# google-research/weatherbenchX

Measured on AMD Instinct MI355X. Metric: grid-point·metric evals/s (0.25° 721×1440×37L) at 1/2/4/8 GPUs; % HBM roofline, higher is better.
Workload: dtype f32+f64

## Files before the change

### weatherbenchx_amd/csrc/wbx_common.hpp

```cpp
#pragma once
#include <hip/hip_runtime.h>

#include <cstdarg>
#include <cstdint>
#include <cstdio>
#include <cstring>

#include "../../include/wbx.h"

struct wbx_ctx {
  int device = 0;
  int num_cus = 256;
  hipStream_t stream = nullptr;
  bool own_stream = false;
  hipEvent_t ev_start = nullptr;
  hipEvent_t ev_stop = nullptr;
  void* fft_state = nullptr;
  void* s2_scratch = nullptr;
  size_t s2_scratch_size = 0;
  void* aidm_scratch = nullptr;
  size_t aidm_scratch_size = 0;
  void* atoms_clean = nullptr;
  void* patch_counters = nullptr;
  size_t patch_counters_size = 0;
  uint32_t ens_queue_parity = 0;
  hipEvent_t* marks = nullptr;
  int marks_used = 0, marks_made = 0, marks_cap = 0;
};

namespace wbx {

char* last_error_buf();

inline int fail(int code, const char* fmt, ...) {
  va_list ap;
  va_start(ap, fmt);
  vsnprintf(last_error_buf(), 512, fmt, ap);
  va_end(ap);
  return code;
}

template <typename T>
__device__ __forceinline__ T ld_stream(const T* p) {
#ifdef WBX_LD_STREAM_PLAIN
  return *p;
#else
  return __builtin_nontemporal_load(p);
#endif
}

__device__ __forceinline__ const char* uniform_ptr(const char* p) {
  const uint64_t v = (uint64_t)p;
  const uint32_t lo = __builtin_amdgcn_readfirstlane((uint32_t)v), hi = __builtin_amdgcn_readfirstlane((uint32_t)(v >> 32));
  return (const char*)(((uint64_t)hi << 32) | lo);
}

template <typename T>
using global_ptr = const __attribute__((address_space(1))) T*;

template <typename T>
using const_ptr = const __attribute__((address_space(4))) T*;

static __constant__ int64_t wbx_zero_i64[1] = {0};
static __constant__ double wbx_one_f64[1] = {1.0};

__device__ __forceinline__ int64_t readlane64(int64_t v, int j) {
  const int lo = __builtin_amdgcn_readlane((int)(uint32_t)(uint64_t)v, j);
  const int hi = __builtin_amdgcn_readlane((int)(uint32_t)((uint64_t)v >> 32), j);
  return (int64_t)(((uint64_t)(uint32_t)hi << 32) | (uint32_t)lo);
}

__device__ __forceinline__ double wave_sum(double v) {
#pragma unroll
  for (int o = 32; o > 0; o >>= 1) v += __shfl_xor(v, o, 64);
  return v;
}

template <int CTRL, int ROW_MASK>
__device__ __forceinline__ double dpp_moved(double v) {
  const int lo = __builtin_amdgcn_update_dpp(0, __double2loint(v), CTRL, ROW_MASK, 0xf, true);
  const int hi = __builtin_amdgcn_update_dpp(0, __double2hiint(v), CTRL, ROW_MASK, 0xf, true);
  return __hiloint2double(hi, lo);
}

__device__ __forceinline__ double wave_sum_lane63(double v) {
  v += dpp_moved<0xB1, 0xf>(v);
  v += dpp_moved<0x4E, 0xf>(v);
  v += dpp_moved<0x124, 0xf>(v);
  v += dpp_moved<0x128, 0xf>(v);
  v += dpp_moved<0x142, 0xa>(v);
  v += dpp_moved<0x143, 0xc>(v);
  return v;
}

__device__ __forceinline__ double wave_sum_uniform(double v) {
  const double t = wave_sum_lane63(v);
  return __hiloint2double(__builtin_amdgcn_readlane(__double2hiint(t), 63), __builtin_amdgcn_readlane(__double2loint(t), 63));
}

}

#define WBX_HIP(expr)                                                                   \
  do {                                                                                  \
    hipError_t _e = (expr);                                                             \
    if (_e != hipSuccess)                                                               \
      return wbx::fail(WBX_ERR_HIP, "%s failed: %s (%s:%d)", #expr, hipGetErrorString(_e), \
                       __FILE__, __LINE__);                                             \
  } while (0)

#define WBX_REQUIRE(cond, ...)                                   \
  do {                                                           \
    if (!(cond)) return wbx::fail(WBX_ERR_INVALID, __VA_ARGS__); \
  } while (0)
```

### weatherbenchx_amd/csrc/wbx_ens_impl.hpp

```cpp
#pragma once
#include <cmath>
#include <cstdlib>

#include "wbx_s1.hpp"
#include "wbx_sortnet_gen.hpp"
#include "wbx_sortnet3_gen.hpp"

#ifndef WBX_ENS_MIN_WAVES
#define WBX_ENS_MIN_WAVES 1
#endif

#ifndef WBX_ENS_MIN_WAVES_PLAIN
#define WBX_ENS_MIN_WAVES_PLAIN WBX_ENS_MIN_WAVES
#endif
#ifndef WBX_ENS_SORTNET3
#define WBX_ENS_SORTNET3 1
#endif

#ifndef WBX_ENS_NOFALLBACK
#define WBX_ENS_NOFALLBACK 0
#endif
#ifndef WBX_ENS_STATS32
#define WBX_ENS_STATS32 1
#endif

namespace wbx {

constexpr int WBX_ENS_DIAG_LOADONLY = 99;
constexpr int WBX_ENS_DIAG_PAIRWISE_LDS = 98;
constexpr int WBX_ENS_SKIPNA_SORT = 97;

template <typename T>
struct EnsOpGeneric {
  static constexpr int NIN = 2;
  static constexpr int NLANE = WBX_ENS_LANES;
  static constexpr int NACC = WBX_ENS_LANES;
  static constexpr int XR_UNROLL = 1, XK_UNROLL = 1, MIN_WAVES = 1;

  __device__ __forceinline__ static void values(const S1Args& a, const int64_t (&ro)[WBX_MAX_INPUTS], int64_t x,
                                                double (&val)[NLANE]) {
    const int M = a.M;
    const T* pp = reinterpret_cast<const T*>(a.in[0]) + ro[0] + x * a.xstride[0];
    const double td = (double)(reinterpret_cast<const T*>(a.in[1])[ro[1] + x * a.xstride[1]]);
    const bool skip = a.flags & WBX_FLAG_SKIPNA_ENS;
    double se = 0.0, sq = 0.0, sabs = 0.0, pair_total = 0.0, x0 = 0.0;
    int n = 0;
    for (int i = 0; i < M; ++i) {
      const double xi = (double)pp[(int64_t)i * a.mstride];
      if (skip && xi != xi) continue;
      if (n == 0) x0 = xi;
      ++n;
      const double e = xi - x0;
      se += e;
      sq = fma(e, e, sq);
      sabs += fabs(xi - td);
      double row = 0.0;
      for (int j = 0; j < i; ++j) {
        const double xj = (double)pp[(int64_t)j * a.mstride];
        if (skip && xj != xj) continue;
        row += fabs(xi - xj);
      }
      pair_total += row;
    }
    const double dM = (double)n;
    const double fair = (a.flags & WBX_FLAG_FAIR) ? 1.0 : 0.0;
    const double mean_e = se / dM;
    const double mean_d = (x0 - td) + mean_e;
    const double var = (sq - se * mean_e) / (dM - 1.0);
    val[0] = sabs / dM;
    val[1] = 2.0 * pair_total / (dM * (dM - fair));
    val[2] = var;
    val[3] = mean_d * mean_d - var / dM;
    val[4] = mean_d * mean_d;
  }

  template <int V, bool XK>
  __device__ __forceinline__ static void accum(const S1Args& a, const int64_t (&ro)[WBX_MAX_INPUTS], int64_t x,
                                               double (&acc)[XK ? V : 1][NACC]) {
    static_assert(V == 1, "ensemble op is one point per lane");
    double val[NLANE];
    values(a, ro, x, val);
#pragma unroll
    for (int l = 0; l < NLANE; ++l) acc[0][l] += val[l];
  }
};

template <int MP, bool EXACT, int ALGO>
struct EnsOpF32 {
  static constexpr int NIN = 2;
  static constexpr int NLANE = WBX_ENS_LANES;
  static constexpr int NACC = WBX_ENS_LANES;
  static constexpr int XR_UNROLL = 1, XK_UNROLL = 1, MIN_WAVES = WBX_ENS_MIN_WAVES_PLAIN;

  struct Regs {
    float xm[MP];
    float t;
    float poison;
  };

  __device__ __forceinline__ static void load(const S1Args& a, const int64_t (&ro)[WBX_MAX_INPUTS], int64_t x, Regs& r) {
    const int M = EXACT ? MP : a.M;
    const float* pp = reinterpret_cast<const float*>(a.in[0]) + ro[0] + x * a.xstride[0];
    r.t = ld_stream(reinterpret_cast<const float*>(a.in[1]) + ro[1] + x * a.xstride[1]);
#pragma unroll
    for (int m = 0; m < MP; ++m) r.xm[m] = (EXACT || m < M) ? ld_stream(pp + (int64_t)m * a.mstride) : INFINITY;
  }

  __device__ __forceinline__ static void values(const S1Args& a, const int64_t (&ro)[WBX_MAX_INPUTS], int64_t x,
                                                double (&val)[NLANE]) {
    Regs r;
    load(a, ro, x, r);
    finish(a, ro, x, r, val);
  }

  template <bool FAST32 = false>
  __device__ __forceinline__ static bool compute(const S1Args& a, Regs& r, double (&val)[NLANE]) {
    const int M = EXACT ? MP : a.M;
    const double td = (double)r.t;
    float(&xm)[MP] = r.xm;

    if constexpr (ALGO == WBX_ENS_DIAG_LOADONLY) {
      float s = 0.f;
#pragma unroll
      for (int m = 0; m < MP; ++m)
        if (EXACT || m < M) s += xm[m];
      val[0] = (double)s - td;
      val[1] = val[2] = val[3] = val[4] = 0.0;
      return false;
    }
    double pair_total = 0.0;
    float poison = 0.f;
    int nvalid = 0;
    bool weird = false;
    float shift32 = 0.f;
    if constexpr (ALGO == WBX_ENS_SKIPNA_SORT) {
      const bool tfin32 = (r.t - r.t) == 0.f;
      shift32 = r.t;
      if (__builtin_amdgcn_ballot_w64(!tfin32)) {
        float lo = INFINITY;
#pragma unroll
        for (int m = 0; m < MP; ++m)
          if (EXACT || m < M) lo = fminf(lo, xm[m]);
        shift32 = tfin32 ? r.t : lo;
      }
#pragma unroll
      for (int m = 0; m < MP; ++m) {
        if (EXACT || m < M) {
          const float x = xm[m];
          const bool missing = x != x;
          nvalid += missing ? 0 : 1;
          xm[m] = missing ? shift32 : x;
        }
      }
      if constexpr (!EXACT) {
        float big = 0.f;
        int m = 0;
        for (; m + 1 < MP; m += 2) {
          const float a = m < M ? xm[m] : 0.f, b = m + 1 < M ? xm[m + 1] : 0.f;
          asm("v_max3_f32 %0, %1, |%2|, |%3|" : "=v"(big) : "v"(big), "v"(a), "v"(b));
        }
        if (m < MP) {
          const float a = m < M ? xm[m] : 0.f;
          asm("v_max3_f32 %0, %1, |%2|, |%2|" : "=v"(big) : "v"(big), "v"(a));
        }
        weird = big == INFINITY;
      }
    }
    if constexpr (ALGO == WBX_ENS_PAIRWISE) {
#pragma unroll
      for (int i = 1; i < MP; ++i) {
        if (EXACT || i < M) {
          float row = 0.f;
#pragma unroll
          for (int j = 0; j < i; ++j) row += fabsf(xm[i] - xm[j]);
          pair_total += (double)row;
        }
      }
    } else if constexpr (ALGO == WBX_ENS_SORT || ALGO == WBX_ENS_SKIPNA_SORT) {
      if constexpr (ALGO == WBX_ENS_SORT) {
        typedef float pk2 __attribute__((ext_vector_type(2)));
        pk2 pz = {0.f, 0.f};
#pragma unroll
        for (int m = 0; m + 1 < MP; m += 2) {
          const pk2 x2 = {xm[m], (EXACT || m + 1 < M) ? xm[m + 1] : 0.f};
          if (EXACT || m < M) pz = x2 * (pk2){0.f, 0.f} + pz;
        }
        if ((MP & 1) && (EXACT || MP - 1 < M)) pz.x = fmaf(xm[MP - 1], 0.f, pz.x);
        poison = pz.x + pz.y;
      }
      auto mn = [](float u, float v) {
        float r;
        asm("v_min_f32 %0, %1, %2" : "=v"(r) : "v"(u), "v"(v));
        return r;
      };
      auto mx = [](float u, float v) {
        float r;
        asm("v_max_f32 %0, %1, %2" : "=v"(r) : "v"(u), "v"(v));
        return r;
      };
      if constexpr (WBX_ENS_SORTNET3) {
        SortNet3<MP>::sort(
            xm, mn, mx,
            [](float u, float v, float w) {
              float r;
              asm("v_min3_f32 %0, %1, %2, %3" : "=v"(r) : "v"(u), "v"(v), "v"(w));
              return r;
            },
            [](float u, float v, float w) {
              float r;
              asm("v_med3_f32 %0, %1, %2, %3" : "=v"(r) : "v"(u), "v"(v), "v"(w));
              return r;
            },
            [](float u, float v, float w) {
              float r;
              asm("v_max3_f32 %0, %1, %2, %3" : "=v"(r) : "v"(u), "v"(v), "v"(w));
              return r;
            });
      } else {
        SortNet<MP>::sort(xm, mn, mx);
      }
    }

    bool redo = false;
    if constexpr (ALGO == WBX_ENS_SKIPNA_SORT) {
      if constexpr (EXACT) weird = xm[0] == -INFINITY || xm[MP - 1] == INFINITY;
      stats_skipna(a, xm, nvalid, td, shift32, val);
      r.poison = 0.f;
      return weird;
    }
    if constexpr (FAST32 && EXACT && ALGO == WBX_ENS_SORT && WBX_ENS_STATS32) {
      const float range = xm[MP - 1] - xm[0];
      const float big = fmaxf(fmaxf(fabsf(xm[0]), fabsf(xm[MP - 1])), fabsf(r.t));
      const bool fast_ok = (range == 0.f || (range >= 0x1p-50f && range <= 0x1p60f)) && big <= 0x1p100f;
      redo = !WBX_ENS_NOFALLBACK && __builtin_amdgcn_ballot_w64(!fast_ok) != 0;
      if (!redo) stats32(a, xm, r.t, poison, val);
      r.poison = poison;
    } else {
      stats64(a, xm, td, pair_total, val);
      r.poison = poison;
      apply_poison(r, val);
    }
    return redo;
  }

  __device__ __forceinline__ static void apply_poison(const Regs& r, double (&val)[NLANE]) {
    if constexpr (ALGO == WBX_ENS_SORT) {
      if (r.poison != r.poison) {
#pragma unroll
        for (int l = 0; l < NLANE; ++l) val[l] = (double)r.poison;
      }
    }
  }

  template <bool FAST32 = false>
  __device__ __forceinline__ static void finish(const S1Args& a, const int64_t (&ro)[WBX_MAX_INPUTS], int64_t x, Regs& r,
                                                double (&val)[NLANE]) {
    if (compute<FAST32>(a, r, val)) {
      EnsOpGeneric<float>::values(a, ro, x, val);
      apply_poison(r, val);
    }
  }

  __device__ __forceinline__ static double recip_small(double n) {
    double r = __builtin_amdgcn_rcp(n);
    r = fma(fma(-n, r, 1.0), r, r);
    r = fma(fma(-n, r, 1.0), r, r);
    return r;
  }
  __device__ __forceinline__ static void stats_skipna(const S1Args& a, const float (&xm)[MP], const int n, const double td,
                                                      const float shift32, double (&val)[NLANE]) {
    const int M = EXACT ? MP : a.M;
    const double shift = (double)shift32;
    const double x0t = shift - td;
    const double dM = (double)n, dK = (double)(M - n);
    double se = 0.0, sq = 0.0, sabs = 0.0, dot1 = 0.0;
#pragma unroll
    for (int m = 0; m < MP; ++m) {
      if (EXACT || m < M) {
        const double e = (double)xm[m] - shift;
        se += e;
        sq = fma(e, e, sq);
        sabs += fabs(e);
        dot1 = fma((double)(2 * m + 1), e, dot1);
      }
    }
    const double dot = fma(-dM, se, fma(-dK, sabs + se, dot1));
    sabs += n > 0 ? fabs(x0t) : 0.0;
    const double nan = __builtin_nan("");
    const double inv_n = n > 0 ? recip_small(dM) : nan;
    const double inv_n1 = n > 1 ? recip_small(dM - 1.0) : nan;
    const double inv_pairs = (a.flags & WBX_FLAG_FAIR) ? inv_n * inv_n1 : inv_n * inv_n;
    const double mean_e = se * inv_n;
    const double mean_d = x0t + mean_e;
    const double var = (sq - se * mean_e) * inv_n1;
    val[0] = sabs * inv_n;
    val[1] = 2.0 * dot * inv_pairs;
    val[2] = var;
    val[3] = mean_d * mean_d - var * inv_n;
    val[4] = mean_d * mean_d;
  }

  __device__ __forceinline__ static void stats64(const S1Args& a, float (&xm)[MP], const double td, const double pair_total,
                                                 double (&val)[NLANE]) {
    const int M = EXACT ? MP : a.M;
    const double x0 = (double)xm[0];
    const bool tfin = (td - td) == 0.0;
    const double shift = tfin ? td : x0;
    const double x0t = shift - td;
    double se = 0.0, sq = 0.0, sabs = 0.0, dot = 0.0;
#pragma unroll
    for (int m = 0; m < MP; ++m) {
      if (EXACT || m < M) {
        const double e = (double)xm[m] - shift;
        se += e;
        sq = fma(e, e, sq);
        sabs += fabs(e);
        if constexpr (ALGO == WBX_ENS_SORT) dot = fma((double)(2 * (m + 1) - M - 1), e, dot);
      }
    }
    sabs += fabs(x0t);
    const double dM = (double)M;
    const double fair = (a.flags & WBX_FLAG_FAIR) ? 1.0 : 0.0;
    const double inv_m = 1.0 / dM, inv_m1 = 1.0 / (dM - 1.0), spread_scale = 2.0 / (dM * (dM - fair));
    const double mean_e = se * inv_m;
    const double mean_d = x0t + mean_e;
    const double var = (sq - se * mean_e) * inv_m1;
    double spread;
    if constexpr (ALGO == WBX_ENS_SORT) {
      spread = dot * spread_scale;
    } else {
      spread = pair_total * spread_scale;
    }
    if constexpr (ALGO == WBX_ENS_DIAG_PAIRWISE_LDS) {
      static_assert(EXACT && MP % 17 == 0, "the LDS-tiled diagnostic is instantiated for M = 51");
      constexpr int B = 17, NB = MP / B;
      __shared__ float tile[MP][64];
      float* col = &tile[0][threadIdx.x];
#pragma unroll
      for (int m = 0; m < MP; ++m) col[m * 64] = xm[m];
      asm volatile("" ::: "memory");
      double total = 0.0;
#pragma unroll
      for (int bi = 0; bi < NB; ++bi) {
        float xi[B];
#pragma unroll
        for (int k = 0; k < B; ++k) xi[k] = col[(bi * B + k) * 64];
#pragma unroll
        for (int k = 1; k < B; ++k) {
          float row = 0.f;
#pragma unroll
          for (int l = 0; l < k; ++l) row += fabsf(xi[k] - xi[l]);
          total += (double)row;
        }
#pragma unroll
        for (int bj = 0; bj < bi; ++bj) {
          float xj[B];
#pragma unroll
          for (int l = 0; l < B; ++l) xj[l] = col[(bj * B + l) * 64];
#pragma unroll
          for (int k = 0; k < B; ++k) {
            float row = 0.f;
#pragma unroll
            for (int l = 0; l < B; ++l) row += fabsf(xi[k] - xj[l]);
            total += (double)row;
          }
        }
      }
      spread = total * spread_scale;
    }
    val[0] = sabs * inv_m;
    val[1] = spread;
    val[2] = var;
    val[3] = mean_d * mean_d - var * inv_m;
    val[4] = mean_d * mean_d;
  }

  __device__ __forceinline__ static void stats32(const S1Args& a, float (&xm)[MP], const float t, const float poison,
                                                 double (&val)[NLANE]) {
    static_assert(EXACT, "fp32 chain sums are instantiated for the exact-M buckets");
    constexpr int K = 8, MID = MP / 2, NPAIR = MP / 2;
    const float c = xm[MID];
    float se[K], sq[K], sa[K], dt[K];
#pragma unroll
    for (int k = 0; k < K; ++k) se[k] = sq[k] = sa[k] = dt[k] = k == 0 ? poison : 0.f;
#pragma unroll
    for (int i = 0; i < NPAIR; ++i) {
      const int j = MP - 1 - i, k = i % K;
      const float ei = xm[i] - c, ej = xm[j] - c;
      se[k] += ei + ej;
      sq[k] = fmaf(ei, ei, sq[k]);
      sq[k] = fmaf(ej, ej, sq[k]);
      sa[k] += fabsf(xm[i] - t);
      sa[k] += fabsf(xm[j] - t);
      dt[k] = fmaf((float)(MP - 1 - 2 * i), xm[j] - xm[i], dt[k]);
    }
    if constexpr (MP & 1) {
      sa[NPAIR % K] += fabsf(c - t);
    } else {
    }
    auto fold = [](const float (&v)[K]) {
      return ((double)(v[0] + v[4]) + (double)(v[1] + v[5])) + ((double)(v[2] + v[6]) + (double)(v[3] + v[7]));
    };
    const double dse = fold(se), dsq = fold(sq), dsa = fold(sa), ddt = fold(dt);
    constexpr double dM = (double)MP;
    const double fair = (a.flags & WBX_FLAG_FAIR) ? 1.0 : 0.0;
    constexpr double inv_m = 1.0 / dM, inv_m1 = 1.0 / (dM - 1.0);
    const double spread_scale = 2.0 / (dM * (dM - fair));
    const double mean_e = dse * inv_m;
    const double mean_d = ((double)c - (double)t) + mean_e;
    const double var = (dsq - dse * mean_e) * inv_m1;
    val[0] = dsa * inv_m;
    val[1] = ddt * spread_scale;
    val[2] = var;
    val[3] = mean_d * mean_d - var * inv_m;
    val[4] = mean_d * mean_d;
  }

  template <int V, bool XK>
  __device__ __forceinline__ static void accum(const S1Args& a, const int64_t (&ro)[WBX_MAX_INPUTS], int64_t x,
                                               double (&acc)[XK ? V : 1][NACC]) {
    static_assert(V == 1, "ensemble op is one point per lane");
    double val[NLANE];
    values(a, ro, x, val);
#pragma unroll
    for (int l = 0; l < NLANE; ++l) acc[0][l] += val[l];
  }
};

template <class Core, bool SKIPNA>
struct EnsMasked {
  static constexpr int NIN = Core::NIN;
  static constexpr int NLANE = Core::NLANE;
  static constexpr int NACC = Core::NLANE + (SKIPNA ? Core::NLANE : 1);
  static constexpr int XR_UNROLL = 1, XK_UNROLL = 1, MIN_WAVES = WBX_ENS_MIN_WAVES;

  __device__ __forceinline__ static void values(const S1Args& a, const int64_t (&ro)[WBX_MAX_INPUTS], int64_t x,
                                                double (&val)[NLANE]) {
    Core::values(a, ro, x, val);
  }

  template <int V, bool XK>
  __device__ __forceinline__ static void accum(const S1Args& a, const int64_t (&ro)[WBX_MAX_INPUTS], int64_t x,
                                               double (&acc)[XK ? V : 1][NACC]) {
    static_assert(V == 1, "ensemble op is one point per lane");
    double val[NLANE];
    Core::values(a, ro, x, val);
    const bool valid =
        (a.flags & WBX_FLAG_MASKED) ? reinterpret_cast<const uint8_t*>(a.in[3])[ro[3] + x * a.xstride[3]] != 0 : true;
    if constexpr (!SKIPNA) {
#pragma unroll
      for (int l = 0; l < NLANE; ++l) acc[0][l] += valid ? val[l] : 0.0;
      acc[0][NLANE] += valid ? 1.0 : 0.0;
    } else {
#pragma unroll
      for (int l = 0; l < NLANE; ++l) {
        const bool ok = valid && !(val[l] != val[l]);
        acc[0][l] += ok ? val[l] : 0.0;
        acc[0][NLANE + l] += ok ? 1.0 : 0.0;
      }
    }
  }
};


#pragma clang diagnostic push
#pragma clang diagnostic ignored "-Winline-asm"
#ifndef WBX_ENS_PIPE_NLDS
#define WBX_ENS_PIPE_NLDS 50
#endif
#ifndef WBX_ENS_PIPE_WAVES
#define WBX_ENS_PIPE_WAVES 3
#endif
#ifndef WBX_ENS_PIPE_SKIPNA_WAVES
#define WBX_ENS_PIPE_SKIPNA_WAVES 3
#endif
template <int MP, bool EXACT, int ALGO, bool FLAT>
__global__ void __launch_bounds__(64, ALGO == WBX_ENS_SKIPNA_SORT ? WBX_ENS_PIPE_SKIPNA_WAVES : WBX_ENS_PIPE_WAVES)
ens_pipe_kernel(S1Args a, int R) {
  using Op = EnsOpF32<MP, EXACT, ALGO>;
  constexpr int NA = Op::NACC;
  constexpr int NLDS = MP < WBX_ENS_PIPE_NLDS ? MP : WBX_ENS_PIPE_NLDS;
  constexpr int NREG = MP - NLDS;
  __shared__ float stage[NLDS][64];
  const int lane = threadIdx.x;
  const int M = EXACT ? MP : a.M;
  const int64_t b = blockIdx.x;
  const int64_t key = b / a.nchunk;
  const int chunk = (int)(b - key * a.nchunk);
  const int64_t d0 = (int64_t)chunk * a.dchunk;
  const int64_t d1 = d0 + a.dchunk < a.D ? d0 + a.dchunk : a.D;
  const int nx = (int)a.nx;
  const uint32_t lds0 = (uint32_t)(uintptr_t)(__attribute__((address_space(3))) void*)&stage[0][0];
  const int64_t mstride_b = a.mstride * 4;

  int64_t kb[WBX_MAX_INPUTS], ro[WBX_MAX_INPUTS];
  key_bases<2>(a, key, kb);
  double acc[NA];
#pragma unroll
  for (int l = 0; l < NA; ++l) acc[l] = 0.0;

  int64_t d = d0, e0 = 0, e1 = 0, et = 0;
  int wm = 0;
  const int wstep = 64 % nx;
  auto open_segment = [&]() {
    if constexpr (FLAT) {
      const int64_t plane = d / R;
      const int64_t j0 = d - plane * R;
      const int64_t nj = d1 - d < R - j0 ? d1 - d : R - j0;
      row_bases<2>(a, kb, key, plane * R, ro);
      e0 = j0 * nx;
      e1 = (j0 + nj) * nx;
      et = e0 & ~(int64_t)63;
      wm = (int)((et + lane) % nx);
      d += nj;
    } else {
      row_bases<2>(a, kb, key, d, ro);
      e0 = 0;
      e1 = nx;
      et = 0;
      d += 1;
    }
  };

  float xn[NREG > 0 ? NREG : 1], tn = 0.f;
  double wn = 0.0;
  auto issue = [&]() {
    int64_t e = et + lane;
    e = e < e0 ? e0 : (e < e1 ? e : e1 - 1);
    const uint32_t voff = (uint32_t)e * (uint32_t)a.xstride[0] * 4u;
    const char* um = uniform_ptr(reinterpret_cast<const char*>(a.in[0]) + ro[0] * 4);
#pragma unroll
    for (int m = 0; m < NLDS; ++m) {
      if (EXACT || m < M)
        asm volatile("s_add_u32 m0, %2, %3\n\tglobal_load_lds_dword %0, %1 nt" ::"v"(voff), "s"(um), "s"(lds0), "i"(m * 256)
                     : "memory", "scc", "m0");
      um += mstride_b;
      asm volatile("" : "+s"(um));
    }
    const float* pr = reinterpret_cast<const float*>(a.in[0]) + ro[0] + e * a.xstride[0];
#pragma unroll
    for (int m = NLDS; m < MP; ++m) xn[m - NLDS] = (EXACT || m < M) ? ld_stream(pr + (int64_t)m * a.mstride) : INFINITY;
    tn = ld_stream(reinterpret_cast<const float*>(a.in[1]) + ro[1] + e * a.xstride[1]);
    if constexpr (FLAT) wn = a.xw[wm];
  };

  bool more = d < d1;
  if (more) {
    open_segment();
    issue();
  }
  while (more) {
    typename Op::Regs r;
    asm volatile("s_waitcnt vmcnt(0)" ::: "memory");
#pragma unroll
    for (int m = 0; m < NLDS; ++m) r.xm[m] = (EXACT || m < M) ? stage[m][lane] : INFINITY;
#pragma unroll
    for (int m = NLDS; m < MP; ++m) r.xm[m] = xn[m - NLDS];
    r.t = tn;
    const double wcur = wn;
    const int64_t ecur = et + lane;
    const bool valid = ecur >= e0 && ecur < e1;
    const int64_t xcur = ecur < e0 ? e0 : (ecur < e1 ? ecur : e1 - 1);
    int64_t rocur[WBX_MAX_INPUTS];
#pragma unroll
    for (int i = 0; i < WBX_MAX_INPUTS; ++i) rocur[i] = ro[i];
    const bool full = et >= e0 && et + 64 <= e1;
    et += 64;
    if (et >= e1) {
      more = d < d1;
      if (more) open_segment();
    } else if constexpr (FLAT) {
      wm += wstep;
      wm = wm >= nx ? wm - nx : wm;
    }
    asm volatile("s_waitcnt lgkmcnt(0)" ::: "memory");
    if (more) issue();
    double val[Op::NLANE];
    Op::template finish<true>(a, rocur, xcur, r, val);
    if constexpr (FLAT) {
      if (full) {
#pragma unroll
        for (int l = 0; l < NA; ++l) acc[l] = fma(val[l], wcur, acc[l]);
      } else {
#pragma unroll
        for (int l = 0; l < NA; ++l) acc[l] = fma(valid ? val[l] : 0.0, wcur, acc[l]);
      }
    } else if (full) {
#pragma unroll
      for (int l = 0; l < NA; ++l) acc[l] += val[l];
    } else {
#pragma unroll
      for (int l = 0; l < NA; ++l) acc[l] += valid ? val[l] : 0.0;
    }
  }
#pragma unroll
  for (int l = 0; l < NA; ++l) {
    const double v = wave_sum(acc[l]);
    if (lane == l) a.out[(key * a.nchunk + chunk) * NA + l] = v;
  }
}

#pragma clang diagnostic pop

inline bool ens_pipe_ok(const wbx_s1_plan* plan, const S1Args& a, bool skipna_ens = false) {
  static const bool off = getenv("WBX_ENS_PIPE") && atoi(getenv("WBX_ENS_PIPE")) == 0;
  static const bool off_skipna = getenv("WBX_ENS_PIPE_SKIPNA") && atoi(getenv("WBX_ENS_PIPE_SKIPNA")) == 0;
  if (off || (skipna_ens && off_skipna)) return false;
  if (plan->x_kept || plan->x_weights != nullptr || plan->block_threads != 64) return false;
  if (plan->flags & (WBX_FLAG_MASKED | WBX_FLAG_SKIPNA | (skipna_ens ? 0u : (unsigned)WBX_FLAG_SKIPNA_ENS))) return false;
  if (plan->nx <= 0 || plan->ndepth <= 0 || plan->nkey <= 0) return false;
  if (a.xstride[0] < 0 || a.xstride[1] < 0) return false;
  return (double)plan->nx * (double)a.xstride[0] * 4.0 < 4294967296.0;
}

inline bool ens_pipe_flat_ok(const wbx_s1_plan* plan, const S1Args& a) {
  static const bool off = getenv("WBX_ENS_PIPE") && atoi(getenv("WBX_ENS_PIPE")) == 0;
  if (off) return false;
  if (plan->x_kept || plan->x_weights == nullptr || plan->block_threads != 64 || plan->plane_rows <= 0) return false;
  if (plan->flags & (WBX_FLAG_MASKED | WBX_FLAG_SKIPNA | WBX_FLAG_SKIPNA_ENS)) return false;
  if (plan->nx <= 0 || plan->nx > WBX_XW_MAX || plan->ndepth <= 0 || plan->nkey <= 0 || plan->ndepth % plan->plane_rows != 0) return false;
  if (a.xstride[0] != 1 || a.xstride[1] != 1) return false;
  return (double)plan->nx * (double)plan->plane_rows * 4.0 < 4294967296.0;
}

template <int MP, bool EXACT, int ALGO, bool FLAT = false>
int launch_ens_pipe(wbx_ctx* ctx, const wbx_s1_plan* plan, S1Args& a) {
  const int64_t grid = plan->nkey * plan->nchunk;
  WBX_REQUIRE(grid < (int64_t)1 << 31, "grid too large (%lld blocks)", (long long)grid);
  hipLaunchKernelGGL((ens_pipe_kernel<MP, EXACT, ALGO, FLAT>), dim3((unsigned)grid), dim3(64), 0, ctx->stream, a,
                     FLAT ? plan->plane_rows : 0);
  WBX_HIP(hipGetLastError());
  return 0;
}

template <class Op>
int launch_ens_op(wbx_ctx* ctx, const wbx_s1_plan* plan, S1Args& a, bool map) {
  if (map) return launch_map<Op>(ctx, plan, a);
  if (plan->x_weights != nullptr) {
    WBX_REQUIRE(!(plan->flags & WBX_FLAG_SKIPNA_ENS), "flat x-weighted mode does not take skipna_ensemble");
    if (plan->flags & WBX_FLAG_SKIPNA) return launch_flat_weighted1<EnsMasked<Op, true>>(ctx, plan, a);
    if (plan->flags & WBX_FLAG_MASKED) return launch_flat_weighted1<EnsMasked<Op, false>>(ctx, plan, a);
    return launch_flat_weighted1<Op>(ctx, plan, a);
  }
  if (plan->flags & WBX_FLAG_SKIPNA) return launch_partial<EnsMasked<Op, true>, 1>(ctx, plan, a);
  if (plan->flags & WBX_FLAG_MASKED) return launch_partial<EnsMasked<Op, false>, 1>(ctx, plan, a);
  return launch_partial<Op, 1>(ctx, plan, a);
}

template <int MP, bool EXACT>
int launch_ens_bucket(wbx_ctx* ctx, const wbx_s1_plan* plan, S1Args& a, int algo, bool map) {
  if (!map && algo == WBX_ENS_SORT && ens_pipe_ok(plan, a)) return launch_ens_pipe<MP, EXACT, WBX_ENS_SORT>(ctx, plan, a);
  if (!map && algo == WBX_ENS_SORT && ens_pipe_flat_ok(plan, a)) return launch_ens_pipe<MP, EXACT, WBX_ENS_SORT, true>(ctx, plan, a);
  if (algo == WBX_ENS_SORT) return launch_ens_op<EnsOpF32<MP, EXACT, WBX_ENS_SORT>>(ctx, plan, a, map);
  if (algo == WBX_ENS_DIAG_LOADONLY) {
    if (!EXACT || map) return fail(WBX_ERR_INVALID, "the load-only diagnostic exists for the exact-M partial kernels only");
    return launch_partial<EnsOpF32<MP, EXACT, WBX_ENS_DIAG_LOADONLY>, 1>(ctx, plan, a);
  }
  if (algo == WBX_ENS_DIAG_PAIRWISE_LDS) {
    if constexpr (EXACT && MP == 51) {
      if (map || plan->x_weights != nullptr || (plan->flags & (WBX_FLAG_MASKED | WBX_FLAG_SKIPNA)) || plan->block_threads != 64)
        return fail(WBX_ERR_INVALID, "the LDS-tiled pair-form diagnostic exists for the plain partial kernels with one-wave blocks only");
      return launch_partial<EnsOpF32<MP, EXACT, WBX_ENS_DIAG_PAIRWISE_LDS>, 1>(ctx, plan, a);
    } else {
      return fail(WBX_ERR_INVALID, "the LDS-tiled pair-form diagnostic exists for M = 51 only");
    }
  }
  if (!map && algo == WBX_ENS_SKIPNA_SORT && ens_pipe_ok(plan, a, true)) return launch_ens_pipe<MP, EXACT, WBX_ENS_SKIPNA_SORT>(ctx, plan, a);
  if (algo == WBX_ENS_SKIPNA_SORT) return launch_ens_op<EnsOpF32<MP, EXACT, WBX_ENS_SKIPNA_SORT>>(ctx, plan, a, map);
  return launch_ens_op<EnsOpF32<MP, EXACT, WBX_ENS_PAIRWISE>>(ctx, plan, a, map);
}

int launch_ens_m4(wbx_ctx*, const wbx_s1_plan*, S1Args&, int, bool);
int launch_ens_m8(wbx_ctx*, const wbx_s1_plan*, S1Args&, int, bool);
int launch_ens_m16(wbx_ctx*, const wbx_s1_plan*, S1Args&, int, bool);
int launch_ens_m32(wbx_ctx*, const wbx_s1_plan*, S1Args&, int, bool);
int launch_ens_m64(wbx_ctx*, const wbx_s1_plan*, S1Args&, int, bool);
int launch_ens_m50(wbx_ctx*, const wbx_s1_plan*, S1Args&, int, bool);
int launch_ens_m51(wbx_ctx*, const wbx_s1_plan*, S1Args&, int, bool);

}
```

Baseline: 120.1 billion.

## Cut register and address overhead in ensemble pipeline kernel inner loop

Makes the row offsets wave-uniform with readfirstlane, switches the per-lane element index to 32-bit, and issues the register-resident member and target loads through scalar base pointers plus 32-bit voffsets. It inlines compute instead of calling finish, falling back to the generic path only when compute reports non-finite input. For the exact SORT case it uses builtin med3/min/max sorting primitives and two poison accumulators so the compiler can schedule them. The aim is fewer VGPRs and less 64-bit address arithmetic per iteration. The eligibility check now also covers the target stride so 32-bit offsets stay valid.

```diff
diff --git a/weatherbenchx_amd/csrc/wbx_common.hpp b/weatherbenchx_amd/csrc/wbx_common.hpp
--- a/weatherbenchx_amd/csrc/wbx_common.hpp
+++ b/weatherbenchx_amd/csrc/wbx_common.hpp
@@ -49,10 +49,25 @@
 #endif
 }
 
+template <typename T>
+__device__ __forceinline__ T ld_stream_global(const __attribute__((address_space(1))) T* p) {
+#ifdef WBX_LD_STREAM_PLAIN
+  return *p;
+#else
+  return __builtin_nontemporal_load(p);
+#endif
+}
+
 __device__ __forceinline__ const char* uniform_ptr(const char* p) {
   const uint64_t v = (uint64_t)p;
   const uint32_t lo = __builtin_amdgcn_readfirstlane((uint32_t)v), hi = __builtin_amdgcn_readfirstlane((uint32_t)(v >> 32));
   return (const char*)(((uint64_t)hi << 32) | lo);
+}
+
+__device__ __forceinline__ int64_t uniform_i64(int64_t x) {
+  const uint64_t v = (uint64_t)x;
+  const uint32_t lo = __builtin_amdgcn_readfirstlane((uint32_t)v), hi = __builtin_amdgcn_readfirstlane((uint32_t)(v >> 32));
+  return (int64_t)(((uint64_t)hi << 32) | lo);
 }
 
 template <typename T>
diff --git a/weatherbenchx_amd/csrc/wbx_ens_impl.hpp b/weatherbenchx_amd/csrc/wbx_ens_impl.hpp
--- a/weatherbenchx_amd/csrc/wbx_ens_impl.hpp
+++ b/weatherbenchx_amd/csrc/wbx_ens_impl.hpp
@@ -113,7 +113,7 @@
     finish(a, ro, x, r, val);
   }
 
-  template <bool FAST32 = false>
+  template <bool FAST32 = false, bool VISIBLE = false>
   __device__ __forceinline__ static bool compute(const S1Args& a, Regs& r, double (&val)[NLANE]) {
     const int M = EXACT ? MP : a.M;
     const double td = (double)r.t;
@@ -179,14 +179,19 @@
     } else if constexpr (ALGO == WBX_ENS_SORT || ALGO == WBX_ENS_SKIPNA_SORT) {
       if constexpr (ALGO == WBX_ENS_SORT) {
         typedef float pk2 __attribute__((ext_vector_type(2)));
-        pk2 pz = {0.f, 0.f};
+        constexpr int NC = VISIBLE ? 2 : 1;
+        pk2 pz[NC];
+#pragma unroll
+        for (int c = 0; c < NC; ++c) pz[c] = (pk2){0.f, 0.f};
 #pragma unroll
         for (int m = 0; m + 1 < MP; m += 2) {
           const pk2 x2 = {xm[m], (EXACT || m + 1 < M) ? xm[m + 1] : 0.f};
-          if (EXACT || m < M) pz = x2 * (pk2){0.f, 0.f} + pz;
+          if (EXACT || m < M) pz[(m / 2) % NC] = x2 * (pk2){0.f, 0.f} + pz[(m / 2) % NC];
         }
-        if ((MP & 1) && (EXACT || MP - 1 < M)) pz.x = fmaf(xm[MP - 1], 0.f, pz.x);
-        poison = pz.x + pz.y;
+        if ((MP & 1) && (EXACT || MP - 1 < M)) pz[NC - 1].x = fmaf(xm[MP - 1], 0.f, pz[NC - 1].x);
+#pragma unroll
+        for (int c = 1; c < NC; ++c) pz[0] += pz[c];
+        poison = pz[0].x + pz[0].y;
       }
       auto mn = [](float u, float v) {
         float r;
@@ -198,7 +203,14 @@
         asm("v_max_f32 %0, %1, %2" : "=v"(r) : "v"(u), "v"(v));
         return r;
       };
-      if constexpr (WBX_ENS_SORTNET3) {
+      if constexpr (VISIBLE && WBX_ENS_SORTNET3) {
+        SortNet3<MP>::sort(
+            xm, [](float u, float v) { return __builtin_amdgcn_fmed3f(u, v, -INFINITY); },
+            [](float u, float v) { return __builtin_amdgcn_fmed3f(u, v, INFINITY); },
+            [](float u, float v, float w) { return __builtin_fminf(__builtin_fminf(u, v), w); },
+            [](float u, float v, float w) { return __builtin_amdgcn_fmed3f(u, v, w); },
+            [](float u, float v, float w) { return __builtin_fmaxf(__builtin_fmaxf(u, v), w); });
+      } else if constexpr (WBX_ENS_SORTNET3) {
         SortNet3<MP>::sort(
             xm, mn, mx,
             [](float u, float v, float w) {
@@ -470,6 +482,9 @@
 #endif
 #ifndef WBX_ENS_PIPE_WAVES
 #define WBX_ENS_PIPE_WAVES 3
+#endif
+#ifndef WBX_ENS_PIPE_KNOCK
+#define WBX_ENS_PIPE_KNOCK 0
 #endif
 #ifndef WBX_ENS_PIPE_SKIPNA_WAVES
 #define WBX_ENS_PIPE_SKIPNA_WAVES 3
@@ -520,13 +535,15 @@
       et = 0;
       d += 1;
     }
+#pragma unroll
+    for (int i = 0; i < 2; ++i) ro[i] = uniform_i64(ro[i]);
   };
 
   float xn[NREG > 0 ? NREG : 1], tn = 0.f;
   double wn = 0.0;
   auto issue = [&]() {
-    int64_t e = et + lane;
-    e = e < e0 ? e0 : (e < e1 ? e : e1 - 1);
+    int e = (int)et + lane;
+    e = e < (int)e0 ? (int)e0 : (e < (int)e1 ? e : (int)e1 - 1);
     const uint32_t voff = (uint32_t)e * (uint32_t)a.xstride[0] * 4u;
     const char* um = uniform_ptr(reinterpret_cast<const char*>(a.in[0]) + ro[0] * 4);
 #pragma unroll
@@ -537,10 +554,13 @@
       um += mstride_b;
       asm volatile("" : "+s"(um));
     }
-    const float* pr = reinterpret_cast<const float*>(a.in[0]) + ro[0] + e * a.xstride[0];
-#pragma unroll
-    for (int m = NLDS; m < MP; ++m) xn[m - NLDS] = (EXACT || m < M) ? ld_stream(pr + (int64_t)m * a.mstride) : INFINITY;
-    tn = ld_stream(reinterpret_cast<const float*>(a.in[1]) + ro[1] + e * a.xstride[1]);
+#pragma unroll
+    for (int m = NLDS; m < MP; ++m) {
+      xn[m - NLDS] = (EXACT || m < M) ? ld_stream_global((global_ptr<float>)((global_ptr<char>)um + voff)) : INFINITY;
+      um += mstride_b;
+    }
+    const char* ut = uniform_ptr(reinterpret_cast<const char*>(a.in[1]) + ro[1] * 4);
+    tn = ld_stream_global((global_ptr<float>)((global_ptr<char>)ut + (uint32_t)e * (uint32_t)a.xstride[1] * 4u));
     if constexpr (FLAT) wn = a.xw[wm];
   };
 
@@ -558,12 +578,8 @@
     for (int m = NLDS; m < MP; ++m) r.xm[m] = xn[m - NLDS];
     r.t = tn;
     const double wcur = wn;
-    const int64_t ecur = et + lane;
-    const bool valid = ecur >= e0 && ecur < e1;
-    const int64_t xcur = ecur < e0 ? e0 : (ecur < e1 ? ecur : e1 - 1);
-    int64_t rocur[WBX_MAX_INPUTS];
-#pragma unroll
-    for (int i = 0; i < WBX_MAX_INPUTS; ++i) rocur[i] = ro[i];
+    const int64_t etc = et, e0c = e0, e1c = e1;
+    [[maybe_unused]] const int64_t ro0 = ro[0], ro1 = ro[1];
     const bool full = et >= e0 && et + 64 <= e1;
     et += 64;
     if (et >= e1) {
@@ -576,7 +592,27 @@
     asm volatile("s_waitcnt lgkmcnt(0)" ::: "memory");
     if (more) issue();
     double val[Op::NLANE];
-    Op::template finish<true>(a, rocur, xcur, r, val);
+#if WBX_ENS_PIPE_KNOCK
+    {
+      float s0 = r.t, s1 = 0.f;
+#pragma unroll
+      for (int m = 0; m + 1 < MP; m += 2) s0 += r.xm[m], s1 += r.xm[m + 1];
+      if constexpr (MP & 1) s0 += r.xm[MP - 1];
+      val[0] = (double)(s0 + s1);
+#pragma unroll
+      for (int l = 1; l < Op::NLANE; ++l) val[l] = 0.0;
+    }
+#else
+    if (Op::template compute<true, !FLAT && EXACT && ALGO == WBX_ENS_SORT>(a, r, val)) {
+      const int ecur = (int)etc + lane;
+      const int64_t xcur = ecur < (int)e0c ? (int)e0c : (ecur < (int)e1c ? ecur : (int)e1c - 1);
+      const int64_t rocur[WBX_MAX_INPUTS] = {ro0, ro1, 0, 0};
+      EnsOpGeneric<float>::values(a, rocur, xcur, val);
+      Op::apply_poison(r, val);
+    }
+#endif
+    const int ecur = (int)etc + lane;
+    const bool valid = ecur >= (int)e0c && ecur < (int)e1c;
     if constexpr (FLAT) {
       if (full) {
 #pragma unroll
@@ -610,7 +646,7 @@
   if (plan->flags & (WBX_FLAG_MASKED | WBX_FLAG_SKIPNA | (skipna_ens ? 0u : (unsigned)WBX_FLAG_SKIPNA_ENS))) return false;
   if (plan->nx <= 0 || plan->ndepth <= 0 || plan->nkey <= 0) return false;
   if (a.xstride[0] < 0 || a.xstride[1] < 0) return false;
-  return (double)plan->nx * (double)a.xstride[0] * 4.0 < 4294967296.0;
+  return (double)plan->nx * (double)(a.xstride[0] > a.xstride[1] ? a.xstride[0] : a.xstride[1]) * 4.0 < 4294967296.0;
 }
 
 inline bool ens_pipe_flat_ok(const wbx_s1_plan* plan, const S1Args& a) {
```

Result: faster. 121.3 billion, median of 6 (+1.0%).
